# DavidSlayback/gym-po-taxi

Measured on AMD Instinct MI355X. Metric: env steps/sec (whole node), FourRooms 11x11 Hansen-4 at 1M envs, 1/2/4/8 GPUs, higher is better.
Workload: dtype int32; 1 GPU; configs[1]: FourRooms 11x11 (FR_MAP) Hansen-4 obs, 1048576 envs per GPU, MultistoryFourRoomsEnv(grid_z=1, obs_type='hansen'); envs_per_gpu=1048576, global_envs=1048576, rng_mode=numpy, parallelism=independent env shards x1, steps_per_launch_call=128, kernel_autotune=windowed

## Files before the change

### gym-po-taxi_amd/csrc/wgrid.hip

```cpp
#include <stdint.h>

#include "gp_internal.h"
#include "grid_shared.h"

namespace {

#ifdef GP_STAMPS
constexpr int ST_STEPS = 24, ST_SLOTS = 42;
__shared__ unsigned long long g_stamp[32 * 32 + 8];
#define WSTAMP(P, k, i)                                                                                  \
  do {                                                                                                   \
    if ((threadIdx.x & 63) == 0 && (k) < ST_STEPS) {                                                     \
      unsigned long long t_;                                                                             \
      asm volatile("s_memrealtime %0\n\ts_waitcnt lgkmcnt(0)" : "=s"(t_)::"memory");                     \
      g_stamp[(k) * ST_SLOTS + (i)] = t_;                                                                \
    }                                                                                                    \
  } while (0)
#define LSTAMP(P, i)                                                                                     \
  do {                                                                                                   \
    if ((threadIdx.x & 63) == 0) {                                                                       \
      unsigned long long t_;                                                                             \
      asm volatile("s_memrealtime %0\n\ts_waitcnt lgkmcnt(0)" : "=s"(t_)::"memory");                     \
      g_stamp[32 * 32 + (i)] = t_;                                                                       \
    }                                                                                                    \
  } while (0)
#else
#define WSTAMP(P, k, i) \
  do {                  \
  } while (0)
#define LSTAMP(P, i) \
  do {               \
  } while (0)
#endif

constexpr int TM_NOSTORE = 1;
constexpr int TM_NOFILL = 2;
constexpr int TM_LATEACT = 4;
constexpr int TM_THROTTLE = 8;
constexpr int TM_BUSYPOLL = 16;
constexpr int TM_NOPRIO = 32;
constexpr int TM_EAGERSTORE = 64;
constexpr int TM_NOCAND = 128;
constexpr int TM_STORELOW = 256;
constexpr int TM_ENVHIGH = 512;
constexpr int TM_NOTABLES = 1024;
constexpr int TM_NOFIRST = 2048;
constexpr int TM_ACTSTART = 4096;
constexpr int TM_OLDPRO = 8192;
constexpr int TM_CELLSWAP = 16384;

constexpr int EW = 8;
#ifndef WG_SW
#define WG_SW 2
#endif
constexpr int SW = WG_SW;
constexpr int CWAVE = EW;
constexpr int NWAVES = EW + 1 + SW;
constexpr int TPB = NWAVES * 64;
constexpr int NL = EW * 64;
constexpr int SLICE = 62;
constexpr int MAXRP = 512;
constexpr int NCAND = 512;
constexpr uint32_t CAND_W = 192;

struct WgShared {
  uint64_t mask[8][EW];
  uint32_t trans_done;
  uint32_t cs_done;
  uint32_t r2s_done;
  uint32_t fill_done;
  uint32_t res_done;
  uint32_t st_done;
  uint32_t sx_ready;
  uint32_t sy_ready;
  uint32_t cells_done;
  uint32_t pro;
  uint64_t sx[2][2];
  uint64_t sy[2][2];
  uint64_t rw[2][2];
  int32_t rw_off[2];
  uint32_t fix[2];
  uint32_t R, h, u, nrp;
  uint32_t cbase;
  uint32_t rp[MAXRP];
  uint16_t r2s[4096];
  uint16_t cand[NCAND];
};

__device__ __forceinline__ void lds_barrier() {
  __builtin_amdgcn_fence(__ATOMIC_RELEASE, "workgroup", "local");
  __builtin_amdgcn_s_barrier();
  __builtin_amdgcn_fence(__ATOMIC_ACQUIRE, "workgroup", "local");
}
__device__ __forceinline__ void lds_release() { __builtin_amdgcn_fence(__ATOMIC_RELEASE, "workgroup", "local"); }
__device__ __forceinline__ void lds_acquire() { __builtin_amdgcn_fence(__ATOMIC_ACQUIRE, "workgroup", "local"); }
__device__ __forceinline__ uint32_t lds_load(const uint32_t* p) {
  return __hip_atomic_load(p, __ATOMIC_RELAXED, __HIP_MEMORY_SCOPE_WORKGROUP);
}
__device__ __forceinline__ void lds_add(uint32_t* p, uint32_t v) {
  __hip_atomic_fetch_add(p, v, __ATOMIC_RELAXED, __HIP_MEMORY_SCOPE_WORKGROUP);
}
__device__ __forceinline__ void lds_wait(const uint32_t* p, uint32_t want, uint32_t* err) {
  uint32_t n = 0;
  while (lds_load(p) < want) {
    __builtin_amdgcn_s_sleep(1);
    if (++n > (1u << 26)) {
      atomicOr(err, GP_DERR_TIMEOUT);
      break;
    }
  }
  lds_acquire();
}

__device__ __forceinline__ uint32_t wave_incl_scan(uint32_t x) {
  x += (uint32_t)__builtin_amdgcn_update_dpp(0, (int)x, 0x111, 0xF, 0xF, true);
  x += (uint32_t)__builtin_amdgcn_update_dpp(0, (int)x, 0x112, 0xF, 0xF, true);
  x += (uint32_t)__builtin_amdgcn_update_dpp(0, (int)x, 0x114, 0xF, 0xF, true);
  x += (uint32_t)__builtin_amdgcn_update_dpp(0, (int)x, 0x118, 0xF, 0xF, true);
  x += (uint32_t)__builtin_amdgcn_update_dpp(0, (int)x, 0x142, 0xA, 0xF, false);
  x += (uint32_t)__builtin_amdgcn_update_dpp(0, (int)x, 0x143, 0xC, 0xF, false);
  return x;
}
__device__ __forceinline__ uint32_t wave_sum(uint32_t x) {
  return (uint32_t)__builtin_amdgcn_readlane((int)wave_incl_scan(x), 63);
}
__device__ __forceinline__ uint32_t mbcnt(uint64_t m) {
  return __builtin_amdgcn_mbcnt_hi((uint32_t)(m >> 32), __builtin_amdgcn_mbcnt_lo((uint32_t)m, 0u));
}
__device__ __forceinline__ uint64_t ballot(bool p) { return __ballot((int)p); }

__device__ __forceinline__ void words_to_draws(uint32_t wtot, uint32_t h0, uint32_t& used, uint32_t& h) {
  if (wtot == 0) {
    used = 0; h = h0;
  } else if (h0) {
    used = wtot >> 1; h = (wtot - 1) & 1;
  } else {
    used = (wtot + 1) >> 1; h = wtot & 1;
  }
}

__host__ __device__ __forceinline__ uint64_t thr_on_u64(uint64_t t) {
  return t >= (1ull << 53) ? ~0ull : ((t << 11) | 0x7FFull);
}

template <int NA>
__device__ __forceinline__ int32_t action_row(int32_t a, uint32_t* derr) {
  if (action_out_of_range(a, NA)) flag_bad_action(derr);
  if (a < 0) a += NA;
  return min(max(a, 0), NA - 1) * NA * 8;
}

struct Tabs {
  const PcgJump* j32p;
  const PcgJump* jt8p;
  const int32_t* ocp;
  const uint16_t* avp;
  const PcgJump* jt64;
  int32_t halo;
  __device__ __forceinline__ Tabs(const char* d, const WgParams& P)
      : j32p(reinterpret_cast<const PcgJump*>(d + P.lds.j32)), jt8p(reinterpret_cast<const PcgJump*>(d + P.lds.jt8)),
        ocp(reinterpret_cast<const int32_t*>(d + P.lds.ocell)), avp(reinterpret_cast<const uint16_t*>(d + P.lds.avalid)),
        jt64(P.jt64), halo(P.halo) {}
  __device__ __forceinline__ const PcgJump& j32(uint32_t i) const { return j32p[i]; }
  __device__ __forceinline__ const PcgJump& jt8(uint32_t i) const { return jt8p[i]; }
  __device__ __forceinline__ int32_t ocell(uint32_t c) const { return ocp[c]; }
  __device__ __forceinline__ uint32_t avalid(uint32_t v) const { return avp[v]; }
};

__device__ __forceinline__ u128 load_cs(const uint64_t* CS, uint32_t j) {
  const ulonglong2 v = reinterpret_cast<const ulonglong2*>(CS)[j];
  return mk128(v.y, v.x);
}
__device__ __forceinline__ u128 draw_state(const Tabs& tb, const uint64_t* CS, uint32_t d) {
  return apply_jump(tb.j32(d & 31u), load_cs(CS, d >> 5));
}

__device__ __forceinline__ u128 jump_any(const Tabs& tb, u128 s, uint32_t n) {
  if (n < 65536u) {
    if (n & 255u) s = apply_jump(tb.jt8(n & 255u), s);
    if (n >> 8) s = apply_jump(tb.jt8(256u + (n >> 8)), s);
    return s;
  }
  return pcg_jump(tb.jt64, s, n);
}

__device__ __forceinline__ u128 rw_base(const Tabs& tb, const PcgJump& jb, u128 Sx, uint32_t used, int beta,
                                        int32_t& heff) {
  const int32_t H = tb.halo;
  if (beta == 0) {
    heff = min(H, (int32_t)used + 1);
    return apply_jump(jb, jump_any(tb, Sx, used + 1u - (uint32_t)heff));
  }
  heff = H;
  return apply_jump(jb, jump_any(tb, Sx, used + 1u));
}

__device__ __forceinline__ bool spin_give_up(const WgParams& P, uint32_t& spins) {
  ++spins;
  if ((spins & 63u) == 0 &&
      (__hip_atomic_load(&P.ctl->err, __ATOMIC_RELAXED, __HIP_MEMORY_SCOPE_AGENT) & GP_DERR_TIMEOUT))
    return true;
  if (spins > P.spin_limit) {
    atomicOr(&P.ctl->err, GP_DERR_TIMEOUT);
    return true;
  }
  return false;
}

__device__ __forceinline__ uint64_t gran(uint32_t tag, uint32_t rej, uint32_t cnt) {
  return ((uint64_t)tag << 32) | ((uint64_t)min(rej, 255u) << 24) | (uint64_t)(cnt & 0xFFFFFFu);
}
__device__ __forceinline__ void publish(const WgParams& P, uint64_t* slots, uint32_t tag, uint32_t rej, uint32_t cnt) {
  if ((threadIdx.x & 63) == 0 && (int)blockIdx.x != P.fault_block)
    __hip_atomic_store(&slots[blockIdx.x], gran(tag, rej, cnt), __ATOMIC_RELAXED, __HIP_MEMORY_SCOPE_AGENT);
}
__device__ __forceinline__ void gather(const WgParams& P, const uint64_t* slots, uint32_t tag, uint64_t (&g)[4]) {
  const bool nap = !(P.tmode & TM_BUSYPOLL);
  const int lane = threadIdx.x & 63, G = (int)gridDim.x;
  uint32_t pend = 0;
#pragma unroll
  for (int j = 0; j < 4; ++j) {
    g[j] = (uint64_t)tag << 32;
    if (lane * 4 + j < G) pend |= 1u << j;
  }
  uint32_t spins = 0;
  while (true) {
#pragma unroll
    for (int j = 0; j < 4; ++j)
      if (pend & (1u << j)) g[j] = __hip_atomic_load(&slots[lane * 4 + j], __ATOMIC_RELAXED, __HIP_MEMORY_SCOPE_AGENT);
#pragma unroll
    for (int j = 0; j < 4; ++j)
      if ((pend & (1u << j)) && (uint32_t)(g[j] >> 32) == tag) pend &= ~(1u << j);
    if (!__any((int)pend)) break;
    if (spin_give_up(P, spins)) {
#pragma unroll
      for (int j = 0; j < 4; ++j)
        if (pend & (1u << j)) g[j] = (uint64_t)tag << 32;
      break;
    }
    if (nap) __builtin_amdgcn_s_sleep(1);
  }
}
__device__ __forceinline__ void exchange(const WgParams& P, uint64_t* slots, uint32_t tag, uint32_t rej, uint32_t cnt,
                                         uint64_t (&g)[4]) {
  publish(P, slots, tag, rej, cnt);
  gather(P, slots, tag, g);
}

__device__ __forceinline__ uint32_t gcnt(uint64_t g) { return (uint32_t)g & 0xFFFFFFu; }
__device__ __forceinline__ uint32_t grej(uint64_t g) { return (uint32_t)(g >> 24) & 0xFFu; }

#ifndef WG_NSTG
#define WG_NSTG 3
#endif
#ifndef WG_EAGER_TAIL
#define WG_EAGER_TAIL 4
#endif
#ifndef WG_SUNROLL
#define WG_SUNROLL 2
#endif
constexpr int NSTG = WG_NSTG;
struct Lds {
  uint64_t* RW;
  uint64_t* CS0;
  char* stg0;
  __device__ __forceinline__ Lds(char* dyn, const WgParams& P, int E)
      : RW(reinterpret_cast<uint64_t*>(dyn + P.lds.total)),
        CS0(reinterpret_cast<uint64_t*>(dyn + P.lds.total + (size_t)(E + 2 * P.halo) * 8)),
        stg0(dyn + P.lds.total + (size_t)(E + 2 * P.halo) * 8 + 2 * 512 * 16) {}
  __device__ __forceinline__ char* stg(int k, int E) const { return stg0 + (size_t)(k % NSTG) * E * 4; }
  __device__ __forceinline__ uint64_t* CS(int k) const { return CS0 + (size_t)(k & 1) * 1024; }
};

__device__ __forceinline__ void list_slice(const WgParams& P, WgShared& sh, const Tabs& tb, const uint64_t* CS,
                                           uint32_t sigma, u128 Sy, uint32_t h, uint32_t u) {
  const int lane = threadIdx.x & 63;
  bool rlo = false, rhi = false;
  if (lane < SLICE) {
    const uint32_t d = 62u * sigma + (uint32_t)lane;
    const u128 s = d < 16384u ? draw_state(tb, CS, d) : pcg_jump(tb.jt64, Sy, d + 1u);
    const uint64_t x = pcg_output(s);
    rlo = lemire_rejected((uint32_t)x, (uint32_t)P.n_agent, P.thr_agent);
    rhi = lemire_rejected((uint32_t)(x >> 32), (uint32_t)P.n_agent, P.thr_agent);
  }
  const bool rb = sigma == 0 && h && lane == SLICE && lemire_rejected(u, (uint32_t)P.n_agent, P.thr_agent);
  const uint64_t mb = ballot(rb), mlo = ballot(rlo), mhi = ballot(rhi);
  const uint32_t n0 = sh.nrp;
  const uint32_t base = n0 + (mb ? 1u : 0u);
  const uint32_t ex = mbcnt(mlo) + mbcnt(mhi);
  const uint32_t pos = 124u * sigma + 2u * (uint32_t)lane + h;
  if (rb && n0 < (uint32_t)MAXRP) sh.rp[n0] = 0;
  if (rlo && base + ex < (uint32_t)MAXRP) sh.rp[base + ex] = pos;
  if (rhi && base + ex + (rlo ? 1u : 0u) < (uint32_t)MAXRP) sh.rp[base + ex + (rlo ? 1u : 0u)] = pos + 1u;
  const uint32_t n1 = base + (uint32_t)__builtin_popcountll(mlo) + (uint32_t)__builtin_popcountll(mhi);
  __builtin_amdgcn_fence(__ATOMIC_RELEASE, "wavefront", "local");
  __builtin_amdgcn_wave_barrier();
  if (lane == 0) {
    if (n1 > (uint32_t)MAXRP) atomicOr(&P.ctl->err, GP_DERR_OVERFLOW);
    sh.nrp = min(n1, (uint32_t)MAXRP);
  }
  __builtin_amdgcn_fence(__ATOMIC_RELEASE, "wavefront", "local");
  __builtin_amdgcn_wave_barrier();
  __builtin_amdgcn_fence(__ATOMIC_ACQUIRE, "wavefront", "local");
}

__device__ __forceinline__ uint32_t list_flagged(const WgParams& P, WgShared& sh, const Tabs& tb, const uint64_t* CS,
                                                 const uint64_t (&g)[4], uint32_t r, u128 Sy, uint32_t h, uint32_t u) {
  const int G = (int)gridDim.x;
  uint32_t r4[4];
#pragma unroll
  for (int j = 0; j < 4; ++j) r4[j] = grej(g[j]);
  const uint32_t tot = wave_sum(r4[0] + r4[1] + r4[2] + r4[3]);
  uint64_t any = ballot((r4[0] | r4[1] | r4[2] | r4[3]) != 0);
  while (any) {
    const int l = __builtin_ctzll(any);
    any &= any - 1;
#pragma unroll
    for (int j = 0; j < 4; ++j)
      if (__builtin_amdgcn_readlane((int)r4[j], l)) list_slice(P, sh, tb, CS, r * (uint32_t)G + (uint32_t)(4 * l + j), Sy, h, u);
  }
  return tot;
}

__device__ __forceinline__ uint32_t ctrl_slow(const WgParams& P, WgShared& sh, const Tabs& tb, const uint64_t* CS, u128 Sy,
                                              uint32_t h, uint32_t u, uint32_t b, uint32_t ts, const uint64_t (&g0)[4]) {
  const int lane = threadIdx.x & 63, G = (int)gridDim.x, beta = (int)blockIdx.x;
  if (lane == 0) sh.nrp = 0;
  __builtin_amdgcn_fence(__ATOMIC_RELEASE, "wavefront", "local");
  __builtin_amdgcn_wave_barrier();
  uint32_t rtot = list_flagged(P, sh, tb, CS, g0, 0u, Sy, h, u);
  uint32_t covered = 124u * (uint32_t)G;
  uint64_t* slots = P.slots + (size_t)(ts & 1u) * 2 * G;
  for (uint32_t r = 1; covered < b + rtot && r < 64u; ++r) {
    const uint32_t sigma = r * (uint32_t)G + (uint32_t)beta;
    uint32_t rj = 0;
    if (lane < SLICE) {
      const uint64_t x = pcg_output(pcg_jump(tb.jt64, Sy, 62u * sigma + (uint32_t)lane + 1u));
      rj = (lemire_rejected((uint32_t)x, (uint32_t)P.n_agent, P.thr_agent) ? 1u : 0u) +
           (lemire_rejected((uint32_t)(x >> 32), (uint32_t)P.n_agent, P.thr_agent) ? 1u : 0u);
    }
    const uint32_t cnt = wave_sum(rj);
    uint64_t g[4];
    exchange(P, slots + (size_t)(r & 1u) * G, (ts << 6) | r, cnt, 0u, g);
    rtot += list_flagged(P, sh, tb, CS, g, r, Sy, h, u);
    covered += 124u * (uint32_t)G;
  }
  uint32_t wtot = 0;
  if (b) {
    uint32_t p = b - 1u;
    const uint32_t n = sh.nrp;
    for (uint32_t q = 0; q < n; ++q) p += sh.rp[q] <= p ? 1u : 0u;
    wtot = p + 1u;
  }
  return wtot;
}

template <int NS, int NA>
__device__ __forceinline__ void wg_ctrl(const WgParams& P, WgShared& sh, const Tabs& tb, const Lds& L, int K) {
  const int lane = threadIdx.x & 63, beta = (int)blockIdx.x, G = (int)gridDim.x;
  constexpr int E = NS * 512;
  GridCtl* C = P.ctl;
  u128 Sx = mk128(C->s_hi, C->s_lo);
  uint32_t h = C->has_u32, u = C->uinteger;
  uint32_t bprev = C->fb_last;
  uint32_t Rprev = (uint32_t)(((uint64_t)bprev * (uint64_t)blockIdx.x) / (uint64_t)gridDim.x);
  const uint32_t ts0 = C->wstep + 1u;
  const PcgJump jr = P.jrej[(size_t)beta * 64 + lane];
  const PcgJump jb = P.jblk[2 * beta], jpro = P.jblk[2 * beta + 1];
  const PcgJump jB = P.jB;
  const uint32_t nag = (uint32_t)P.n_agent, thra = P.thr_agent;
  const int32_t H = P.halo;
  const uint32_t bias = (uint32_t)P.wg_bias;
  const bool envcells = NS <= 2 && !(P.tmode & TM_CELLSWAP);
  uint32_t* derr = &C->err;
  lds_barrier();
  if (lane == 0 && (P.tmode & TM_OLDPRO)) {
    const u128 s = apply_jump(jpro, Sx);
    sh.rw[0][0] = hi64(s);
    sh.rw[0][1] = lo64(s);
    sh.rw_off[0] = beta == 0 ? 1 : H;
    lds_release();
    __hip_atomic_store(&sh.pro, 1u, __ATOMIC_RELAXED, __HIP_MEMORY_SCOPE_WORKGROUP);
  }
  LSTAMP(P, 1);
  for (int k = 0; k < K; ++k) {
    const uint32_t ts = ts0 + (uint32_t)k;
    if (lane == 0) {
      sh.sx[k & 1][0] = hi64(Sx);
      sh.sx[k & 1][1] = lo64(Sx);
      lds_release();
      __hip_atomic_store(&sh.sx_ready, (uint32_t)k + 1u, __ATOMIC_RELAXED, __HIP_MEMORY_SCOPE_WORKGROUP);
    }
    uint32_t rj = 0;
    if (lane < SLICE) {
      const uint64_t x = pcg_output(apply_jump(jr, Sx));
      rj = (lemire_rejected((uint32_t)x, nag, thra) ? 1u : 0u) + (lemire_rejected((uint32_t)(x >> 32), nag, thra) ? 1u : 0u);
    } else if (lane == SLICE && beta == 0 && h) {
      rj = lemire_rejected(u, nag, thra) ? 1u : 0u;
    }
    const uint32_t rejc = wave_sum(rj);
    WSTAMP(P, k, 6);
    lds_wait(&sh.trans_done, (uint32_t)EW * (uint32_t)(k + 1), derr);
    WSTAMP(P, k, 7);
    const uint32_t cb = wave_sum(lane < NS * EW ? (uint32_t)__builtin_popcountll(sh.mask[lane >> 3][lane & 7]) : 0u);
    uint64_t* slots = P.slots + (size_t)(ts & 1u) * 2 * G;
    publish(P, slots, ts << 6, rejc, cb);
    WSTAMP(P, k, 8);
    const u128 Sy = apply_jump(jB, Sx);
    uint32_t used_p, hp;
    words_to_draws(bprev + bias, h, used_p, hp);
    int32_t heff_p;
    const u128 Srw = rw_base(tb, jb, Sx, used_p, beta, heff_p);
    if (lane == 0) {
      sh.sy[k & 1][0] = hi64(Sy);
      sh.sy[k & 1][1] = lo64(Sy);
      sh.rw[(k + 1) & 1][0] = hi64(Srw);
      sh.rw[(k + 1) & 1][1] = lo64(Srw);
      lds_release();
      __hip_atomic_store(&sh.sy_ready, (uint32_t)k + 1u, __ATOMIC_RELAXED, __HIP_MEMORY_SCOPE_WORKGROUP);
    }
    const uint64_t* CS = L.CS(k);
    lds_wait(&sh.cs_done, (uint32_t)EW * (uint32_t)(k + 1), derr);
    const uint32_t d0 = min(Rprev > CAND_W + h ? (Rprev - CAND_W - h) >> 1 : 0u, 16384u - NCAND / 2);
    const uint32_t cbase = 2u * d0 + h;
    if (!(P.tmode & TM_NOCAND)) {
#pragma unroll
      for (int m = 0; m < NCAND / 128; ++m) {
        const uint32_t j = (uint32_t)(lane + 64 * m);
        const uint64_t x = pcg_output(draw_state(tb, CS, d0 + j));
        sh.cand[2 * j] = (uint16_t)tb.avalid(lemire_value((uint32_t)x, nag));
        sh.cand[2 * j + 1] = (uint16_t)tb.avalid(lemire_value((uint32_t)(x >> 32), nag));
      }
    }
    __builtin_amdgcn_fence(__ATOMIC_RELEASE, "wavefront", "local");
    __builtin_amdgcn_wave_barrier();
    __builtin_amdgcn_fence(__ATOMIC_ACQUIRE, "wavefront", "local");
    uint64_t g[4];
    gather(P, slots, ts << 6, g);
    WSTAMP(P, k, 9);
    const uint32_t bsum = gcnt(g[0]) + gcnt(g[1]) + gcnt(g[2]) + gcnt(g[3]);
    const uint32_t incl = wave_incl_scan(bsum);
    const uint32_t b = (uint32_t)__builtin_amdgcn_readlane((int)incl, 63);
    uint32_t R;
    {
      const int bl = beta >> 2, bj = beta & 3;
      uint32_t before = incl - bsum;
#pragma unroll
      for (int j = 0; j < 4; ++j) before += j < bj ? gcnt(g[j]) : 0u;
      R = (uint32_t)__builtin_amdgcn_readlane((int)before, bl);
    }
    const uint32_t rtot = wave_sum(grej(g[0]) + grej(g[1]) + grej(g[2]) + grej(g[3]));
    const bool slow = rtot != 0 || b > 124u * (uint32_t)G;
    uint32_t used, h2;
    lds_wait(&sh.r2s_done, (uint32_t)EW * (uint32_t)(k + 1), derr);
    if (!slow) {
      words_to_draws(b, h, used, h2);
      if (envcells && lane == 0) {
        sh.R = R;
        sh.h = h;
        sh.u = u;
        sh.cbase = cbase;
      }
      if (cb && !envcells) {
        uint16_t* st = reinterpret_cast<uint16_t*>(L.stg(k, E));
        for (uint32_t q = (uint32_t)lane; q < cb; q += 64u) {
          const uint32_t hw = R + q;
          const uint32_t slot = sh.r2s[q];
          uint32_t cell;
          if (hw - cbase < (uint32_t)NCAND && !(P.tmode & TM_NOCAND)) {
            cell = sh.cand[hw - cbase];
          } else {
            uint32_t word;
            if (h && hw == 0) {
              word = u;
            } else {
              const uint32_t hh = hw - h;
              const uint64_t x = pcg_output(draw_state(tb, CS, hh >> 1));
              word = (hh & 1u) ? (uint32_t)(x >> 32) : (uint32_t)x;
            }
            cell = tb.avalid(lemire_value(word, nag));
          }
          st[2 * slot] = (uint16_t)cell;
        }
      }
    } else {
      const uint32_t wtot = ctrl_slow(P, sh, tb, CS, Sy, h, u, b, ts, g);
      words_to_draws(wtot, h, used, h2);
      if (lane == 0) {
        sh.R = R;
        sh.h = h;
        sh.u = u;
      }
    }
    int32_t off = heff_p + (int32_t)used - (int32_t)used_p;
    uint32_t fix = slow ? 1u : 0u;
    if (k + 1 < K && (off < 0 || off > 2 * H)) {
      int32_t heff;
      const u128 s = rw_base(tb, jb, Sx, used, beta, heff);
      off = heff;
      fix |= 2u;
      if (lane == 0) {
        sh.rw[(k + 1) & 1][0] = hi64(s);
        sh.rw[(k + 1) & 1][1] = lo64(s);
      }
    }
    if (lane == 0) {
      sh.rw_off[(k + 1) & 1] = off;
      sh.fix[k & 1] = fix;
      lds_release();
      __hip_atomic_store(&sh.cells_done, (uint32_t)k + 1u, __ATOMIC_RELAXED, __HIP_MEMORY_SCOPE_WORKGROUP);
    }
    WSTAMP(P, k, 10);
    Sx = jump_any(tb, Sy, used);
    if (used) u = (uint32_t)(pcg_output(Sx) >> 32);
    h = h2;
    bprev = b;
    Rprev = R;
    WSTAMP(P, k, 12);
  }
  LSTAMP(P, 3);
  if (beta == 0 && lane == 0) {
    C->s_hi = hi64(Sx);
    C->s_lo = lo64(Sx);
    C->has_u32 = h;
    C->uinteger = u;
    C->fb_last = bprev;
    C->wstep = ts0 + (uint32_t)K - 1u;
  }
}

struct Acc {
  uint32_t eps = 0, ngoal = 0, nwall = 0, lens = 0;
};

template <int NS>
__device__ __forceinline__ void wg_env_slow(const WgParams& P, WgShared& sh, const Tabs& tb, const uint64_t* CS,
                                            int k, char* stg, uint32_t dn, const uint32_t (&pre)[NS],
                                            const uint64_t (&bm)[NS], uint32_t (&ae)[NS]) {
  const int lg = threadIdx.x;
  const u128 Sy = mk128(sh.sy[k & 1][0], sh.sy[k & 1][1]);
  const uint32_t R = sh.R, h = sh.h, u = sh.u, n = sh.nrp;
#pragma unroll
  for (int s = 0; s < NS; ++s) {
    if (!((dn >> s) & 1u)) continue;
    uint32_t p = R + pre[s] + mbcnt(bm[s]);
    for (uint32_t q = 0; q < n; ++q) p += sh.rp[q] <= p ? 1u : 0u;
    uint32_t word;
    if (h && p == 0) {
      word = u;
    } else {
      const uint32_t hh = p - h, d = hh >> 1;
      const u128 st = d < 16384u ? draw_state(tb, CS, d) : pcg_jump(tb.jt64, Sy, d + 1u);
      const uint64_t x = pcg_output(st);
      word = (hh & 1u) ? (uint32_t)(x >> 32) : (uint32_t)x;
    }
    const uint32_t cell = tb.avalid(lemire_value(word, (uint32_t)P.n_agent));
    reinterpret_cast<uint16_t*>(stg)[2 * (s * 512 + lg)] = (uint16_t)cell;
    ae[s] = cell;
  }
}

template <int NS>
__device__ __forceinline__ void wg_env_cells(const WgParams& P, WgShared& sh, const Tabs& tb, const uint64_t* CS,
                                             char* stg, uint32_t dn, const uint32_t (&pre)[NS], const uint64_t (&bm)[NS],
                                             uint32_t (&ae)[NS]) {
  if (!dn) return;
  const int lg = threadIdx.x;
  const uint32_t R = sh.R, h = sh.h, u = sh.u, cbase = sh.cbase;
  const bool nocand = (P.tmode & TM_NOCAND) != 0;
#pragma unroll
  for (int s = 0; s < NS; ++s) {
    if (!((dn >> s) & 1u)) continue;
    const uint32_t hw = R + pre[s] + mbcnt(bm[s]);
    uint32_t cell;
    if (hw - cbase < (uint32_t)NCAND && !nocand) {
      cell = sh.cand[hw - cbase];
    } else {
      uint32_t word;
      if (h && hw == 0) {
        word = u;
      } else {
        const uint32_t hh = hw - h;
        const uint64_t x = pcg_output(draw_state(tb, CS, hh >> 1));
        word = (hh & 1u) ? (uint32_t)(x >> 32) : (uint32_t)x;
      }
      cell = tb.avalid(lemire_value(word, (uint32_t)P.n_agent));
    }
    reinterpret_cast<uint16_t*>(stg)[2 * (s * 512 + lg)] = (uint16_t)cell;
    ae[s] = cell;
  }
}

__device__ __forceinline__ void fill_window(uint64_t* RW, const PcgJump& jl, const PcgJump& jrow, int fr0, int nrow,
                                            u128 base, int lane) {
  u128 s = apply_jump(jl, base);
  uint64_t* d = RW + fr0 * 64 + lane;
  for (int m = 0; m < nrow; ++m) {
    d[m * 64] = pcg_output(s);
    s = apply_jump(jrow, s);
  }
}

template <int NS, int NA>
__device__ __forceinline__ void wg_env(const WgParams& P, WgShared& sh, const Tabs& tb, const Lds& L, const char* dyn,
                                       const int32_t* __restrict__ act, int K, Acc& acc, int32_t* __restrict__ obs,
                                       float* __restrict__ rew, uint8_t* __restrict__ term,
                                       uint8_t* __restrict__ trunc) {
  const int lg = threadIdx.x, lane = lg & 63, w = lg >> 6;
  const int beta = (int)blockIdx.x, G = (int)gridDim.x;
  constexpr int E = NS * 512;
  const size_t B = (size_t)E * (size_t)G;
  const size_t e0 = (size_t)beta * E;
  const char* thr = dyn + P.lds.thr;
  const char* mv = dyn + P.lds.move;
  const uint32_t goal = (uint32_t)P.goal, tlim = (uint32_t)P.time_limit;
  uint32_t* derr = &P.ctl->err;
  uint32_t* aeg = P.ae;
  const bool envcells = NS <= 2 && !(P.tmode & TM_CELLSWAP);
  const int fr0 = P.fill_row0[w], nrow = P.fill_rows[w];
  const int tmode = P.tmode;
  const PcgJump jrow = P.jrow;
  const PcgJump jrw = P.jlane[2 * lg], jcs = P.jlane[2 * lg + 1];
  uint32_t ae[NS];
  int32_t arow[NS], anext[NS];
#pragma unroll
  for (int k = 0; k < NS; ++k) {
    ae[k] = aeg[e0 + (size_t)k * 512 + lg];
    anext[k] = act[e0 + (size_t)k * 512 + lg];
  }
  const bool oldpro = (tmode & TM_OLDPRO) != 0;
  if (!(tmode & TM_NOFIRST)) {
    const GridCtl* C = P.ctl;
    const u128 S0 = mk128(C->s_hi, C->s_lo);
    if (oldpro) {
      fill_window(L.RW, jrw, jrow, fr0, nrow, apply_jump(P.jblk[2 * beta + 1], S0), lane);
    } else {
      const int32_t off0 = beta == 0 ? 1 : P.halo;
      u128 st = apply_jump(P.jfirst[(beta ? 512 : 0) + lg], apply_jump(P.jblk[2 * beta + 1], S0));
      const PcgJump j512 = P.j512;
#pragma unroll
      for (int k = 0; k < NS; ++k) {
        L.RW[k * 512 + lg + off0] = pcg_output(st);
        if (k + 1 < NS) st = apply_jump(j512, st);
      }
      if (lg == 0) sh.rw_off[0] = off0;
    }
  }
  if (w == 0) LSTAMP(P, 2);
  lds_barrier();
#pragma unroll
  for (int k = 0; k < NS; ++k) {
    arow[k] = action_row<NA>(anext[k], derr);
    acc.lens += ae[k] >> 16;
  }
  if (oldpro) {
    lds_wait(&sh.pro, 1u, derr);
    if (lane == 0) lds_add(&sh.fill_done, 1u);
  }
  if (w == 0) LSTAMP(P, 7);
  uint32_t fill_target = EW;
  uint64_t bm[NS];
  uint32_t pre[NS];
  for (int k = 0; k < K; ++k) {
    char* stg = L.stg(k, E);
    if (w == 0) WSTAMP(P, k, 41);
    if (k + 1 < K && !(tmode & (TM_LATEACT | TM_ACTSTART))) {
#pragma unroll
      for (int s = 0; s < NS; ++s) anext[s] = act[(size_t)(k + 1) * B + e0 + (size_t)s * 512 + lg];
    }
    if (w == 0) WSTAMP(P, k, 40);
    lds_wait(&sh.fill_done, fill_target, derr);
    if (k >= NSTG) lds_wait(&sh.st_done, (uint32_t)SW * (uint32_t)(k - NSTG + 1), derr);
    if (!(tmode & TM_NOPRIO)) __builtin_amdgcn_s_setprio(2);
    if (w == 0) WSTAMP(P, k, 0);
    WSTAMP(P, k, 32 + w);
    if (k + 1 < K && (tmode & TM_ACTSTART)) {
#pragma unroll
      for (int s = 0; s < NS; ++s) anext[s] = act[(size_t)(k + 1) * B + e0 + (size_t)s * 512 + lg];
    }
    const int32_t off = sh.rw_off[k & 1];
    uint32_t dn = 0;
    uint32_t mvo[NS];
#pragma unroll
    for (int s = 0; s < NS; ++s) {
      const uint64_t x = L.RW[s * 512 + lg + off];
      const char* t = thr + arow[s];
      uint32_t eb = 0;
#pragma unroll
      for (int j = 0; j + 1 < NA; j += 2) {
        const ulonglong2 tt = *reinterpret_cast<const ulonglong2*>(t + 8 * j);
        eb = x > tt.x ? (uint32_t)(2 * (j + 1)) : eb;
        if (j + 2 < NA) eb = x > tt.y ? (uint32_t)(2 * (j + 2)) : eb;
      }
      mvo[s] = (ae[s] & 0xFFFFu) * (2 * NA) + eb;
    }
    uint32_t mm[NS];
#pragma unroll
    for (int s = 0; s < NS; ++s) mm[s] = *reinterpret_cast<const uint16_t*>(mv + mvo[s]);
    uint32_t sv[NS];
#pragma unroll
    for (int s = 0; s < NS; ++s) {
      const uint32_t m = mm[s];
      const uint32_t nc = m & 0x7FFFu, blocked = m >> 15;
      const uint32_t el = (ae[s] >> 16) + 1u;
      const bool term = nc == goal, trunc = el > tlim, done = term || trunc;
      sv[s] = nc | ((uint32_t)term << 16) | ((uint32_t)trunc << 17) | (blocked << 18);
      ae[s] = done ? nc : (nc | (el << 16));
      bm[s] = ballot(done);
      dn |= (uint32_t)done << s;
      acc.ngoal += term ? 1u : 0u;
      acc.nwall += (blocked && !term) ? 1u : 0u;
    }
    if (lane == 0) {
#pragma unroll
      for (int s = 0; s < NS; ++s) sh.mask[s][w] = bm[s];
    }
#pragma unroll
    for (int s = 0; s < NS; ++s) reinterpret_cast<uint32_t*>(stg)[s * 512 + lg] = sv[s];
    acc.eps += (uint32_t)__builtin_popcount(dn);
    lds_release();
    if (lane == 0) lds_add(&sh.trans_done, 1u);
    if (!(tmode & TM_NOPRIO) && !(tmode & TM_ENVHIGH)) __builtin_amdgcn_s_setprio(0);
    if (w == 0) WSTAMP(P, k, 1);
    WSTAMP(P, k, 16 + w);
    if (k + 1 < K && (tmode & TM_LATEACT)) {
#pragma unroll
      for (int s = 0; s < NS; ++s) anext[s] = act[(size_t)(k + 1) * B + e0 + (size_t)s * 512 + lg];
    }
    lds_wait(&sh.sx_ready, (uint32_t)k + 1u, derr);
    if (w == 0) WSTAMP(P, k, 2);
    {
      const u128 cs = apply_jump(jcs, mk128(sh.sx[k & 1][0], sh.sx[k & 1][1]));
      reinterpret_cast<ulonglong2*>(L.CS(k))[lg] = ulonglong2{lo64(cs), hi64(cs)};
    }
    lds_release();
    if (lane == 0) lds_add(&sh.cs_done, 1u);
    if (w == 0) WSTAMP(P, k, 3);
    lds_wait(&sh.trans_done, (uint32_t)EW * (uint32_t)(k + 1), derr);
    {
      const uint32_t c = lane < NS * EW ? (uint32_t)__builtin_popcountll(sh.mask[lane >> 3][lane & 7]) : 0u;
      const uint32_t ex = wave_incl_scan(c) - c;
#pragma unroll
      for (int s = 0; s < NS; ++s) {
        pre[s] = (uint32_t)__builtin_amdgcn_readlane((int)ex, s * EW + w);
        if ((dn >> s) & 1u) sh.r2s[pre[s] + mbcnt(bm[s])] = (uint16_t)(s * 512 + lg);
      }
    }
    lds_release();
    if (lane == 0) lds_add(&sh.r2s_done, 1u);
    if (w == 0) WSTAMP(P, k, 4);
    if (k + 1 < K) {
      lds_wait(&sh.sy_ready, (uint32_t)k + 1u, derr);
      const u128 Srw = mk128(sh.rw[(k + 1) & 1][0], sh.rw[(k + 1) & 1][1]);
      if (!(tmode & TM_NOFILL)) fill_window(L.RW, jrw, jrow, fr0, nrow, Srw, lane);
      lds_release();
      if (lane == 0) lds_add(&sh.fill_done, 1u);
      fill_target += EW;
#pragma unroll
      for (int s = 0; s < NS; ++s) arow[s] = action_row<NA>(anext[s], derr);
    }
    if (w == 0) WSTAMP(P, k, 5);
    if (w == EW - 1) WSTAMP(P, k, 15);
    WSTAMP(P, k, 24 + w);
    lds_wait(&sh.cells_done, (uint32_t)k + 1u, derr);
    if (w == 0) WSTAMP(P, k, 11);
    const uint32_t fix = sh.fix[k & 1];
    if (fix & 1u) {
      wg_env_slow<NS>(P, sh, tb, L.CS(k), k, stg, dn, pre, bm, ae);
    } else if (envcells) {
      wg_env_cells<NS>(P, sh, tb, L.CS(k), stg, dn, pre, bm, ae);
    } else {
#pragma unroll
      for (int s = 0; s < NS; ++s)
        if ((dn >> s) & 1u) ae[s] = reinterpret_cast<const uint16_t*>(stg)[2 * (s * 512 + lg)];
    }
    lds_release();
    if (lane == 0) lds_add(&sh.res_done, 1u);
    if (k == K - 1 && !(tmode & TM_NOSTORE)) {
      const uint32_t* st = reinterpret_cast<const uint32_t*>(stg);
      const size_t base = (size_t)k * B + e0 + (size_t)lg;
#pragma unroll
      for (int s = 0; s < NS; ++s) {
        const uint32_t v = st[s * 512 + lg];
        const size_t e = base + (size_t)s * 512;
        obs[e] = tb.ocell(v & 0xFFFFu);
        rew[e] = (v & 0x10000u) ? P.r_goal : ((v & 0x40000u) ? P.r_wall : P.r_step);
        term[e] = (uint8_t)((v >> 16) & 1u);
        trunc[e] = (uint8_t)((v >> 17) & 1u);
      }
    }
    if ((fix & 2u) && k + 1 < K) {
      fill_window(L.RW, jrw, jrow, fr0, nrow, mk128(sh.rw[(k + 1) & 1][0], sh.rw[(k + 1) & 1][1]), lane);
      lds_release();
      if (lane == 0) lds_add(&sh.fill_done, 1u);
      fill_target += EW;
    }
  }
#pragma unroll
  for (int k = 0; k < NS; ++k) {
    aeg[e0 + (size_t)k * 512 + lg] = ae[k];
    acc.lens -= ae[k] >> 16;
  }
}

typedef uint32_t u32x4 __attribute__((ext_vector_type(4)));
__device__ __forceinline__ void nt_store(void* p, u32x4 v) { __builtin_nontemporal_store(v, reinterpret_cast<u32x4*>(p)); }

template <int NS>
__device__ __forceinline__ void wg_store(const WgParams& P, WgShared& sh, const Tabs& tb, const Lds& L, int K,
                                         int32_t* __restrict__ obs, float* __restrict__ rew, uint8_t* __restrict__ term,
                                         uint8_t* __restrict__ trunc) {
  const int sl = (int)threadIdx.x - (EW + 1) * 64;
  const int lane = sl & 63;
  const int beta = (int)blockIdx.x, G = (int)gridDim.x;
  constexpr int E = NS * 512;
  const size_t B = (size_t)E * (size_t)G;
  const float rs = P.r_step, rwall = P.r_wall, rg = P.r_goal;
  const int tmode = P.tmode;
  uint32_t* derr = &P.ctl->err;
  lds_barrier();
  for (int k = 0; k + 1 < K; ++k) {
    lds_wait(&sh.res_done, (uint32_t)EW * (uint32_t)(k + 1), derr);
    if (k + WG_EAGER_TAIL < K && !(tmode & TM_EAGERSTORE))
      lds_wait(&sh.trans_done, (uint32_t)EW * (uint32_t)(k + 2), derr);
    if (sl < 64) WSTAMP(P, k, 13);
    const uint32_t* st = reinterpret_cast<const uint32_t*>(L.stg(k, E));
    const size_t base = (size_t)k * B + (size_t)beta * E;
#if WG_SUNROLL == 4
#pragma unroll 4
#elif WG_SUNROLL == 1
#pragma unroll 1
#else
#pragma unroll 2
#endif
    for (int c = sl; c < E / 4 && !(tmode & TM_NOSTORE); c += SW * 64) {
      const uint4 x = reinterpret_cast<const uint4*>(st)[c];
      const uint32_t v[4] = {x.x, x.y, x.z, x.w};
      u32x4 o, r;
      uint32_t tm = 0, tr = 0;
#pragma unroll
      for (int z = 0; z < 4; ++z) {
        o[z] = (uint32_t)tb.ocell(v[z] & 0xFFFFu);
        const float rr = (v[z] & 0x10000u) ? rg : ((v[z] & 0x40000u) ? rwall : rs);
        r[z] = __builtin_bit_cast(uint32_t, rr);
        tm |= ((v[z] >> 16) & 1u) << (8 * z);
        tr |= ((v[z] >> 17) & 1u) << (8 * z);
      }
      const size_t e = base + (size_t)c * 4;
      nt_store(obs + e, o);
      nt_store(rew + e, r);
      __builtin_nontemporal_store(tm, reinterpret_cast<uint32_t*>(term + e));
      __builtin_nontemporal_store(tr, reinterpret_cast<uint32_t*>(trunc + e));
      if (tmode & TM_THROTTLE) asm volatile("s_waitcnt vmcnt(0)" ::: "memory");
    }
    lds_release();
    if (lane == 0) lds_add(&sh.st_done, 1u);
    if (sl < 64) WSTAMP(P, k, 14);
  }
}

template <int NS, int NA>
__global__ __launch_bounds__(TPB) void wgrid_rollout(const WgParams* __restrict__ Pp, int K, const int32_t* __restrict__ act,
                                                      int32_t* __restrict__ obs, float* __restrict__ rew,
                                                      uint8_t* __restrict__ term, uint8_t* __restrict__ trunc) {
  __shared__ WgShared sh;
  extern __shared__ __attribute__((aligned(16))) char dyn[];
  asm volatile("" : "+s"(K));
  const WgParams& P = *Pp;
  const int tid = threadIdx.x, lane = tid & 63, wid = tid >> 6;
  constexpr int E = NS * 512;
  if (tid == 0) LSTAMP(P, 0);
  if (wid >= EW && !(P.tmode & TM_NOTABLES)) {
    constexpr int CT = (NWAVES - EW) * 64;
    const int t = tid - EW * 64;
    const int n = P.lds.total >> 4;
    const uint4* s = reinterpret_cast<const uint4*>(P.limg);
    uint4* d = reinterpret_cast<uint4*>(dyn);
    for (int i0 = t; i0 < n; i0 += 4 * CT) {
      uint4 v0, v1, v2, v3;
      const bool a1 = i0 + CT < n, a2 = i0 + 2 * CT < n, a3 = i0 + 3 * CT < n;
      v0 = s[i0];
      if (a1) v1 = s[i0 + CT];
      if (a2) v2 = s[i0 + 2 * CT];
      if (a3) v3 = s[i0 + 3 * CT];
      d[i0] = v0;
      if (a1) d[i0 + CT] = v1;
      if (a2) d[i0 + 2 * CT] = v2;
      if (a3) d[i0 + 3 * CT] = v3;
    }
    if (wid == EW) LSTAMP(P, 5);
    if (wid == EW + 1) LSTAMP(P, 6);
  }
  if (tid == EW * 64) {
    sh.trans_done = sh.cs_done = sh.r2s_done = sh.fill_done = sh.res_done = sh.st_done = 0;
    sh.sx_ready = sh.sy_ready = sh.cells_done = sh.pro = 0;
    if (!(P.tmode & TM_OLDPRO)) sh.fill_done = EW;
    sh.fix[0] = sh.fix[1] = 0;
  }
  const Tabs tb(dyn, P);
  const Lds L(dyn, P, E);
  Acc acc;
  if (wid == CWAVE) {
    __builtin_amdgcn_s_setprio(3);
    wg_ctrl<NS, NA>(P, sh, tb, L, K);
  } else if (wid > CWAVE) {
    if (P.tmode & TM_STORELOW) __builtin_amdgcn_s_setprio(0);
    else __builtin_amdgcn_s_setprio(1);
    wg_store<NS>(P, sh, tb, L, K, obs, rew, term, trunc);
  } else {
    wg_env<NS, NA>(P, sh, tb, L, dyn, act, K, acc, obs, rew, term, trunc);
  }
  float rsum = 0.f;
  uint32_t nst = 0;
  if (wid < EW) {
    const uint32_t steps = (uint32_t)(NS * K);
    acc.lens += steps;
    nst = steps;
    rsum = (float)acc.ngoal * P.r_goal + (float)acc.nwall * P.r_wall + (float)(steps - acc.ngoal - acc.nwall) * P.r_step;
  }
#pragma unroll
  for (int d = 32; d >= 1; d >>= 1) {
    rsum += __shfl_xor(rsum, d, 64);
    acc.eps += __shfl_xor(acc.eps, d, 64);
    acc.lens += __shfl_xor(acc.lens, d, 64);
    nst += __shfl_xor(nst, d, 64);
  }
  __shared__ float m_r[NWAVES];
  __shared__ uint32_t m_e[NWAVES], m_l[NWAVES], m_n[NWAVES];
  if (lane == 0) {
    m_r[wid] = rsum;
    m_e[wid] = acc.eps;
    m_l[wid] = acc.lens;
    m_n[wid] = nst;
  }
  __syncthreads();
  if (tid == 0) {
    float rr = 0;
    uint32_t e = 0, l = 0, n = 0;
    for (int w = 0; w < NWAVES; ++w) {
      rr += m_r[w];
      e += m_e[w];
      l += m_l[w];
      n += m_n[w];
    }
    MetricSlot& m = P.mslot[blockIdx.x];
    atomicAdd(&m.return_sum, (double)rr);
    atomicAdd(&m.episodes, (unsigned long long)e);
    atomicAdd(&m.length_sum, (unsigned long long)l);
    atomicAdd(&m.env_steps, (unsigned long long)n);
  }
#ifdef GP_STAMPS
  __syncthreads();
  for (int i = tid; i < 32 * 32; i += TPB) P.dbg[(size_t)blockIdx.x * 32 * 32 + i] = g_stamp[i];
  if (tid < 8 && tid != 4) P.dbg[(size_t)256 * 32 * 32 + (size_t)blockIdx.x * 8 + tid] = g_stamp[32 * 32 + tid];
  if (tid == 0) {
    unsigned long long t_;
    asm volatile("s_memrealtime %0\n\ts_waitcnt lgkmcnt(0)" : "=s"(t_)::"memory");
    P.dbg[(size_t)256 * 32 * 32 + (size_t)blockIdx.x * 8 + 4] = t_;
  }
#endif
}

template <int NS, int NA>
void launch_one(const WgArgs& a, int G, size_t lds, hipStream_t s) {
  hipLaunchKernelGGL((wgrid_rollout<NS, NA>), dim3((unsigned)G), dim3(TPB), lds, s, a.P, a.K, a.act, a.obs, a.rew,
                     a.term, a.trunc);
}
template <int NS, int NA>
int fits_one(size_t lds) {
  int occ = 0;
  if (hipOccupancyMaxActiveBlocksPerMultiprocessor(&occ, wgrid_rollout<NS, NA>, TPB, lds) != hipSuccess) return 0;
  return occ;
}

}

int wgrid_launch(const WgArgs& a, int NS, int NA, int G, size_t lds, hipStream_t s) {
  switch (NS * 16 + NA) {
    case 1 * 16 + 4: launch_one<1, 4>(a, G, lds, s); break;
    case 2 * 16 + 4: launch_one<2, 4>(a, G, lds, s); break;
    case 4 * 16 + 4: launch_one<4, 4>(a, G, lds, s); break;
    case 8 * 16 + 4: launch_one<8, 4>(a, G, lds, s); break;
    case 1 * 16 + 8: launch_one<1, 8>(a, G, lds, s); break;
    case 2 * 16 + 8: launch_one<2, 8>(a, G, lds, s); break;
    case 4 * 16 + 8: launch_one<4, 8>(a, G, lds, s); break;
    case 8 * 16 + 8: launch_one<8, 8>(a, G, lds, s); break;
    default: return (int)hipErrorInvalidValue;
  }
  return (int)hipGetLastError();
}

int wgrid_fits(int NS, int NA, size_t lds) {
  switch (NS * 16 + NA) {
    case 1 * 16 + 4: return fits_one<1, 4>(lds);
    case 2 * 16 + 4: return fits_one<2, 4>(lds);
    case 4 * 16 + 4: return fits_one<4, 4>(lds);
    case 8 * 16 + 4: return fits_one<8, 4>(lds);
    case 1 * 16 + 8: return fits_one<1, 8>(lds);
    case 2 * 16 + 8: return fits_one<2, 8>(lds);
    case 4 * 16 + 8: return fits_one<4, 8>(lds);
    case 8 * 16 + 8: return fits_one<8, 8>(lds);
  }
  return 0;
}
```

Measured before the change: 195.2 billion env-steps/s.

## Drop r2s scatter and barrier; control wave walks done-masks directly

The env waves no longer compute a prefix scan and scatter a rank-to-slot table into LDS, and the control wave no longer waits on an r2s_done counter. Instead the control wave scans the per-wave done masks itself, publishes exclusive prefixes in a double-buffered pre array, and walks set bits of each mask with ctz to find slots. Masks are double-buffered by step parity so env waves can proceed to the next step without clobbering them. This removes a cross-wave synchronization point and an LDS scatter. In exchange, the control wave's slot loop becomes per-lane bit iteration, which may be less balanced across lanes.

Measured after the change: 207.8 billion env-steps/s (median of 6 runs). 1.06x the previous value.

```diff
diff --git a/gym-po-taxi_amd/csrc/wgrid.hip b/gym-po-taxi_amd/csrc/wgrid.hip
--- a/gym-po-taxi_amd/csrc/wgrid.hip
+++ b/gym-po-taxi_amd/csrc/wgrid.hip
@@ -64,10 +64,9 @@
 constexpr uint32_t CAND_W = 192;
 
 struct WgShared {
-  uint64_t mask[8][EW];
+  uint64_t mask[2][8][EW];
   uint32_t trans_done;
   uint32_t cs_done;
-  uint32_t r2s_done;
   uint32_t fill_done;
   uint32_t res_done;
   uint32_t st_done;
@@ -83,7 +82,7 @@
   uint32_t R, h, u, nrp;
   uint32_t cbase;
   uint32_t rp[MAXRP];
-  uint16_t r2s[4096];
+  uint32_t pre[2][64];
   uint16_t cand[NCAND];
 };
 
@@ -399,13 +398,6 @@
       rj = lemire_rejected(u, nag, thra) ? 1u : 0u;
     }
     const uint32_t rejc = wave_sum(rj);
-    WSTAMP(P, k, 6);
-    lds_wait(&sh.trans_done, (uint32_t)EW * (uint32_t)(k + 1), derr);
-    WSTAMP(P, k, 7);
-    const uint32_t cb = wave_sum(lane < NS * EW ? (uint32_t)__builtin_popcountll(sh.mask[lane >> 3][lane & 7]) : 0u);
-    uint64_t* slots = P.slots + (size_t)(ts & 1u) * 2 * G;
-    publish(P, slots, ts << 6, rejc, cb);
-    WSTAMP(P, k, 8);
     const u128 Sy = apply_jump(jB, Sx);
     uint32_t used_p, hp;
     words_to_draws(bprev + bias, h, used_p, hp);
@@ -419,6 +411,22 @@
       lds_release();
       __hip_atomic_store(&sh.sy_ready, (uint32_t)k + 1u, __ATOMIC_RELAXED, __HIP_MEMORY_SCOPE_WORKGROUP);
     }
+    WSTAMP(P, k, 6);
+    lds_wait(&sh.trans_done, (uint32_t)EW * (uint32_t)(k + 1), derr);
+    WSTAMP(P, k, 7);
+    uint64_t m = lane < NS * EW ? sh.mask[k & 1][lane >> 3][lane & 7] : 0ull;
+    uint32_t ex;
+    uint32_t cb;
+    {
+      const uint32_t c = (uint32_t)__builtin_popcountll(m);
+      const uint32_t incl = wave_incl_scan(c);
+      ex = incl - c;
+      cb = (uint32_t)__builtin_amdgcn_readlane((int)incl, 63);
+    }
+    uint64_t* slots = P.slots + (size_t)(ts & 1u) * 2 * G;
+    publish(P, slots, ts << 6, rejc, cb);
+    WSTAMP(P, k, 8);
+    sh.pre[k & 1][lane] = ex;
     const uint64_t* CS = L.CS(k);
     lds_wait(&sh.cs_done, (uint32_t)EW * (uint32_t)(k + 1), derr);
     const uint32_t d0 = min(Rprev > CAND_W + h ? (Rprev - CAND_W - h) >> 1 : 0u, 16384u - NCAND / 2);
@@ -452,7 +460,6 @@
     const uint32_t rtot = wave_sum(grej(g[0]) + grej(g[1]) + grej(g[2]) + grej(g[3]));
     const bool slow = rtot != 0 || b > 124u * (uint32_t)G;
     uint32_t used, h2;
-    lds_wait(&sh.r2s_done, (uint32_t)EW * (uint32_t)(k + 1), derr);
     if (!slow) {
       words_to_draws(b, h, used, h2);
       if (envcells && lane == 0) {
@@ -463,9 +470,11 @@
       }
       if (cb && !envcells) {
         uint16_t* st = reinterpret_cast<uint16_t*>(L.stg(k, E));
-        for (uint32_t q = (uint32_t)lane; q < cb; q += 64u) {
-          const uint32_t hw = R + q;
-          const uint32_t slot = sh.r2s[q];
+        const uint32_t seg = (uint32_t)(lane >> 3) * 512u + (uint32_t)(lane & 7) * 64u;
+        while (m) {
+          const uint32_t slot = seg + (uint32_t)__builtin_ctzll(m);
+          m &= m - 1;
+          const uint32_t hw = R + ex++;
           uint32_t cell;
           if (hw - cbase < (uint32_t)NCAND && !(P.tmode & TM_NOCAND)) {
             cell = sh.cand[hw - cbase];
@@ -535,7 +544,7 @@
 
 template <int NS>
 __device__ __forceinline__ void wg_env_slow(const WgParams& P, WgShared& sh, const Tabs& tb, const uint64_t* CS,
-                                            int k, char* stg, uint32_t dn, const uint32_t (&pre)[NS],
+                                            int k, char* stg, uint32_t dn, const uint32_t* prew,
                                             const uint64_t (&bm)[NS], uint32_t (&ae)[NS]) {
   const int lg = threadIdx.x;
   const u128 Sy = mk128(sh.sy[k & 1][0], sh.sy[k & 1][1]);
@@ -543,7 +552,7 @@
 #pragma unroll
   for (int s = 0; s < NS; ++s) {
     if (!((dn >> s) & 1u)) continue;
-    uint32_t p = R + pre[s] + mbcnt(bm[s]);
+    uint32_t p = R + prew[s * EW] + mbcnt(bm[s]);
     for (uint32_t q = 0; q < n; ++q) p += sh.rp[q] <= p ? 1u : 0u;
     uint32_t word;
     if (h && p == 0) {
@@ -562,7 +571,7 @@
 
 template <int NS>
 __device__ __forceinline__ void wg_env_cells(const WgParams& P, WgShared& sh, const Tabs& tb, const uint64_t* CS,
-                                             char* stg, uint32_t dn, const uint32_t (&pre)[NS], const uint64_t (&bm)[NS],
+                                             char* stg, uint32_t dn, const uint32_t* prew, const uint64_t (&bm)[NS],
                                              uint32_t (&ae)[NS]) {
   if (!dn) return;
   const int lg = threadIdx.x;
@@ -571,7 +580,7 @@
 #pragma unroll
   for (int s = 0; s < NS; ++s) {
     if (!((dn >> s) & 1u)) continue;
-    const uint32_t hw = R + pre[s] + mbcnt(bm[s]);
+    const uint32_t hw = R + prew[s * EW] + mbcnt(bm[s]);
     uint32_t cell;
     if (hw - cbase < (uint32_t)NCAND && !nocand) {
       cell = sh.cand[hw - cbase];
@@ -660,7 +669,6 @@
   if (w == 0) LSTAMP(P, 7);
   uint32_t fill_target = EW;
   uint64_t bm[NS];
-  uint32_t pre[NS];
   for (int k = 0; k < K; ++k) {
     char* stg = L.stg(k, E);
     if (w == 0) WSTAMP(P, k, 41);
@@ -713,7 +721,7 @@
     }
     if (lane == 0) {
 #pragma unroll
-      for (int s = 0; s < NS; ++s) sh.mask[s][w] = bm[s];
+      for (int s = 0; s < NS; ++s) sh.mask[k & 1][s][w] = bm[s];
     }
 #pragma unroll
     for (int s = 0; s < NS; ++s) reinterpret_cast<uint32_t*>(stg)[s * 512 + lg] = sv[s];
@@ -736,21 +744,10 @@
     lds_release();
     if (lane == 0) lds_add(&sh.cs_done, 1u);
     if (w == 0) WSTAMP(P, k, 3);
-    lds_wait(&sh.trans_done, (uint32_t)EW * (uint32_t)(k + 1), derr);
-    {
-      const uint32_t c = lane < NS * EW ? (uint32_t)__builtin_popcountll(sh.mask[lane >> 3][lane & 7]) : 0u;
-      const uint32_t ex = wave_incl_scan(c) - c;
-#pragma unroll
-      for (int s = 0; s < NS; ++s) {
-        pre[s] = (uint32_t)__builtin_amdgcn_readlane((int)ex, s * EW + w);
-        if ((dn >> s) & 1u) sh.r2s[pre[s] + mbcnt(bm[s])] = (uint16_t)(s * 512 + lg);
-      }
-    }
-    lds_release();
-    if (lane == 0) lds_add(&sh.r2s_done, 1u);
-    if (w == 0) WSTAMP(P, k, 4);
     if (k + 1 < K) {
+      lds_wait(&sh.trans_done, (uint32_t)EW * (uint32_t)(k + 1), derr);
       lds_wait(&sh.sy_ready, (uint32_t)k + 1u, derr);
+      if (w == 0) WSTAMP(P, k, 4);
       const u128 Srw = mk128(sh.rw[(k + 1) & 1][0], sh.rw[(k + 1) & 1][1]);
       if (!(tmode & TM_NOFILL)) fill_window(L.RW, jrw, jrow, fr0, nrow, Srw, lane);
       lds_release();
@@ -765,10 +762,11 @@
     lds_wait(&sh.cells_done, (uint32_t)k + 1u, derr);
     if (w == 0) WSTAMP(P, k, 11);
     const uint32_t fix = sh.fix[k & 1];
+    const uint32_t* prew = &sh.pre[k & 1][w];
     if (fix & 1u) {
-      wg_env_slow<NS>(P, sh, tb, L.CS(k), k, stg, dn, pre, bm, ae);
+      wg_env_slow<NS>(P, sh, tb, L.CS(k), k, stg, dn, prew, bm, ae);
     } else if (envcells) {
-      wg_env_cells<NS>(P, sh, tb, L.CS(k), stg, dn, pre, bm, ae);
+      wg_env_cells<NS>(P, sh, tb, L.CS(k), stg, dn, prew, bm, ae);
     } else {
 #pragma unroll
       for (int s = 0; s < NS; ++s)
@@ -892,7 +890,7 @@
     if (wid == EW + 1) LSTAMP(P, 6);
   }
   if (tid == EW * 64) {
-    sh.trans_done = sh.cs_done = sh.r2s_done = sh.fill_done = sh.res_done = sh.st_done = 0;
+    sh.trans_done = sh.cs_done = sh.fill_done = sh.res_done = sh.st_done = 0;
     sh.sx_ready = sh.sy_ready = sh.cells_done = sh.pro = 0;
     if (!(P.tmode & TM_OLDPRO)) sh.fill_done = EW;
     sh.fix[0] = sh.fix[1] = 0;
```
